# schulter/crbm

Hardware: AMD Instinct MI355X
Metric: Gibbs-steps/sec (PCD-1) at batch 8192x4x200, 10 motifs len 15 (higher is better)
Workload: dtype f32; 1 GPU; cfg2: 10 motifs len 15, batch 8192 x 4x200, PCD-1, single-stranded; chains_per_gpu=8192, gibbs_steps_per_launch=1, visible=4x200, hidden=10x186, parallelism=chains sharded over 1 GPU(s), no collective in the Gibbs step

## Files before the change

__graft_entry__.py:

```python
import os
import sys

ROOT = os.path.dirname(os.path.abspath(__file__))
if ROOT not in sys.path:
    sys.path.insert(0, ROOT)


PRECOMPILE = [dict(num_motifs=k, motif_length=m, doublestranded=ds) for (k, m, ds) in [
    (10, 15, 0), (10, 15, 1), (50, 25, 0), (20, 15, 1),
    (10, 5, 1), (10, 5, 0), (3, 4, 1), (4, 5, 1), (4, 5, 0), (6, 9, 1), (2, 5, 1),
]]
PRECOMPILE += [dict(num_motifs=6, motif_length=7, doublestranded=1, pooling=2, fantasy_hidden_len=24),
               dict(num_motifs=10, motif_length=15, doublestranded=0, pooling=4, fantasy_hidden_len=48),
               dict(num_motifs=5, motif_length=8, doublestranded=1, pooling=3, fantasy_hidden_len=36)]
PRECOMPILE += [dict(num_motifs=100, motif_length=15, doublestranded=0), dict(num_motifs=20, motif_length=40, doublestranded=1)]
PRECOMPILE += [dict(num_motifs=300, motif_length=10, doublestranded=0, fantasy_hidden_len=51), dict(num_motifs=120, motif_length=40, doublestranded=1, fantasy_hidden_len=61),
               dict(num_motifs=256, motif_length=4, doublestranded=1, fantasy_hidden_len=37), dict(num_motifs=300, motif_length=10, doublestranded=0, batchsize=4096, fantasy_hidden_len=191)]
PRECOMPILE += [dict(num_motifs=300, motif_length=10, doublestranded=0, batchsize=512, fantasy_hidden_len=30),
               dict(num_motifs=120, motif_length=40, doublestranded=1, batchsize=256, fantasy_hidden_len=24)]
PRECOMPILE += [dict(num_motifs=10, motif_length=15, doublestranded=0, batchsize=8192, fantasy_hidden_len=186),
               dict(num_motifs=50, motif_length=25, doublestranded=0, batchsize=8192, fantasy_hidden_len=976),
               dict(num_motifs=20, motif_length=15, doublestranded=1, batchsize=8192, fantasy_hidden_len=486)]
PRECOMPILE += [dict(num_motifs=3, motif_length=3, doublestranded=1, batchsize=4, fantasy_hidden_len=8),
               dict(num_motifs=4, motif_length=4, doublestranded=0, batchsize=4, fantasy_hidden_len=8)]

STATISTICS_SHAPES = [dict(num_motifs=k, motif_length=m, doublestranded=ds, pooling=pool, batchsize=7, fantasy_hidden_len=lf)
                     for (k, m, ds, pool, lf) in [
    (10, 15, 0, 1, 33), (16, 16, 1, 1, 33), (16, 32, 0, 1, 33), (32, 16, 0, 1, 33), (8, 12, 1, 1, 33), (20, 15, 1, 1, 33),
    (33, 17, 0, 1, 33), (64, 32, 1, 1, 33), (20, 40, 1, 1, 33), (4, 64, 1, 1, 33), (100, 15, 0, 1, 33), (130, 7, 1, 1, 33),
    (256, 4, 0, 1, 33), (6, 7, 1, 2, 34), (10, 15, 0, 4, 36), (5, 8, 1, 3, 33), (300, 10, 0, 1, 33), (150, 6, 1, 2, 34),
    (10, 15, 0, 1, 64), (10, 15, 0, 1, 32), (20, 40, 1, 1, 64), (20, 40, 1, 1, 32)]]
GEOMETRY_SHAPES = [dict(num_motifs=k, motif_length=m, doublestranded=ds, batchsize=b, fantasy_hidden_len=lf,
                        env=dict(CRBM_GEOM="2", CRBM_GIBBS_S=str(s)))
                   for (k, m, ds, lf, b, s) in [(10, 15, 0, 186, 8, 4), (10, 15, 0, 185, 8, 4), (10, 15, 0, 185, 6, 2), (10, 15, 1, 50, 6, 2), (40, 6, 0, 30, 4, 4),
                                                (10, 15, 0, 186, 9, 4), (10, 15, 1, 50, 8, 2)]]


def build():
    from crbm_amd.csrc import build as hip_build
    hip_build.build(verbose=True)
    hip_build.prune_cache()
    hip_build.precompile(PRECOMPILE + STATISTICS_SHAPES + GEOMETRY_SHAPES, verbose=False)
    from oracle import build_cpu
    build_cpu.build(verbose=True)
    import crbm_amd
    from crbm_amd import _lib
    lib = _lib.load()
    assert lib.crbm_abi_version() == _lib.ABI_VERSION
    print("crbm_amd", crbm_amd.__version__, "ABI", lib.crbm_abi_version())


def smoke():
    import numpy as np
    from crbm_amd import CRBM
    from oracle.crbm_oracle import OracleCRBM, synthetic_onehot

    K, M, B, Lf, n, L = 10, 15, 64, 186, 48, 200
    W = np.random.default_rng(42).standard_normal((K, 1, 4, M)).astype(np.float32)
    model = CRBM(K, M, doublestranded=False, batchsize=B, cd_k=1, fantasy_hidden_len=Lf, seed=2026)
    oracle = OracleCRBM(K, M, doublestranded=False, batchsize=B, cd_k=1, fantasy_hidden_len=Lf, seed=2026, W=W)
    b = (oracle.b + 4.0).astype(np.float32)
    model.motifs.set_value(W)
    model.bias.set_value(b)
    oracle.b = b.astype(np.float64)
    D = synthetic_onehot(n, L, seed=1234)
    model._trainingFct(D)
    oracle.train_step(D)
    np.testing.assert_allclose(model.motifs.get_value(), oracle.W, rtol=1e-4, atol=2e-6)
    np.testing.assert_allclose(model.bias.get_value(), oracle.b, rtol=1e-4, atol=2e-6)
    np.testing.assert_allclose(model.c.get_value(), oracle.c, rtol=1e-4, atol=2e-6)
    from oracle.crbm_oracle import hidden_uniforms, visible_uniforms, KIND_CHAIN_H, KIND_CHAIN_V
    model.set_fantasy(oracle.fantasy_h.astype(np.float32))
    idx = np.arange(B) + oracle.seq_offset
    for _ in range(3):
        t = oracle.gibbs_step
        model.set_rng(gibbs_step=t)
        uv = visible_uniforms(oracle.seed, t, idx, Lf + M - 1, KIND_CHAIN_V)
        Pv, v = oracle._computeVgivenH(oracle.fantasy_h, None, uv)
        uh = hidden_uniforms(oracle.seed, t, idx, K, Lf, 0, KIND_CHAIN_H)
        P, hnew = oracle._computeHgivenV(v, False, uh)
        model.gibbsSteps(1)
        h, _ = model.get_fantasy()
        gv = model.get_fantasy_visible()
        badv = (gv != v).any(axis=2)[:, 0]
        if badv.any():
            gap = np.min(np.abs(np.cumsum(Pv[:, 0], axis=1)[:, :3] - uv[:, None, :]), axis=1)
            assert np.all(gap[badv] < 1e-6), "visible sample differs away from a tie"
        bad = (h != hnew) & ~badv.any(axis=1)[:, None, None, None]
        assert np.all(np.abs(P - uh)[bad] < 1e-6), "hidden sample differs away from a tie"
        oracle.fantasy_h, oracle.gibbs_step = hnew, t + 1
        model.set_fantasy(hnew.astype(np.float32))
    assert oracle.fantasy_h.sum() > 0
    np.testing.assert_allclose(model.freeEnergy(D), oracle.freeEnergy(D), rtol=1e-4)
    print("smoke ok: train step, Gibbs chain and free energy match the oracle")


if __name__ == "__main__":
    build()
    if os.path.exists("/dev/kfd"):
        smoke()
```

crbm_amd/csrc/crbm_kernels.h:

```cpp
#pragma once
#include <hip/hip_runtime.h>
#include <stdint.h>
#include "crbm_layout.h"

namespace crbm {

template <int I>
struct IC {
  static constexpr int value = I;
};

struct Philox4 {
  uint32_t v[4];
};

struct HalfFrag {
  uint32_t r[4];
};
#if defined(__clang__)
typedef float floatx4 __attribute__((ext_vector_type(4)));
__device__ __forceinline__ uint32_t xor3(uint32_t a, uint32_t b, uint32_t c) { return __builtin_amdgcn_bitop3_b32(a, b, c, 0x96); }
__device__ __forceinline__ uint32_t bitrev32(uint32_t x) { return __builtin_bitreverse32(x); }
__device__ __forceinline__ void store4_streaming(uint32_t* dst, uint32_t x, uint32_t y, uint32_t z, uint32_t w) {
  typedef uint32_t u4v __attribute__((ext_vector_type(4)));
  const u4v val = {x, y, z, w};
  __builtin_nontemporal_store(val, reinterpret_cast<u4v*>(dst));
}
__device__ __forceinline__ void store1_streaming(uint32_t* dst, uint32_t x) { __builtin_nontemporal_store(x, dst); }
__device__ __forceinline__ void wait_vector_memory() { __builtin_amdgcn_s_waitcnt(0x0F70); }
__device__ __forceinline__ float load_system(const float* p) { return __hip_atomic_load(p, __ATOMIC_RELAXED, __HIP_MEMORY_SCOPE_SYSTEM); }
__device__ __forceinline__ uint32_t load_system(const uint32_t* p) { return __hip_atomic_load(p, __ATOMIC_RELAXED, __HIP_MEMORY_SCOPE_SYSTEM); }
__device__ __forceinline__ void store_system(float* p, float v) { __hip_atomic_store(p, v, __ATOMIC_RELAXED, __HIP_MEMORY_SCOPE_SYSTEM); }
__device__ __forceinline__ void store_system(uint32_t* p, uint32_t v) { __hip_atomic_store(p, v, __ATOMIC_RELAXED, __HIP_MEMORY_SCOPE_SYSTEM); }
__device__ __forceinline__ void fence_system() { __threadfence_system(); }
__device__ __forceinline__ void fence_acquire_system() { __builtin_amdgcn_fence(__ATOMIC_ACQUIRE, ""); }
__device__ __forceinline__ uint32_t ticket_add(uint32_t* p) { return __hip_atomic_fetch_add(p, 1u, __ATOMIC_ACQ_REL, __HIP_MEMORY_SCOPE_AGENT); }
__device__ __forceinline__ void short_sleep() { __builtin_amdgcn_s_sleep(8); }
__device__ __forceinline__ uint64_t realtime_ticks() { return __builtin_amdgcn_s_memrealtime(); }
__device__ __forceinline__ uint64_t shader_cycles() { return __builtin_amdgcn_s_memtime(); }
__device__ __forceinline__ void split_f16(const float (&x)[8], HalfFrag& hi, HalfFrag& lo) {
  typedef _Float16 half8 __attribute__((ext_vector_type(8)));
  half8 h, l;
#pragma unroll
  for (int e = 0; e < 8; ++e) {
    h[e] = (_Float16)x[e];
    l[e] = (_Float16)(x[e] - (float)h[e]);
  }
  hi = __builtin_bit_cast(HalfFrag, h);
  lo = __builtin_bit_cast(HalfFrag, l);
}
__device__ __forceinline__ floatx4 mfma_16x16x32_f16(const HalfFrag& a, const HalfFrag& b, floatx4 c) {
  typedef _Float16 half8 __attribute__((ext_vector_type(8)));
  return __builtin_amdgcn_mfma_f32_16x16x32_f16(__builtin_bit_cast(half8, a), __builtin_bit_cast(half8, b), c, 0, 0, 0);
}
typedef float floatx2 __attribute__((vector_size(8)));
__device__ __forceinline__ floatx2 fma2(floatx2 a, floatx2 b, floatx2 c) { return __builtin_elementwise_fma(a, b, c); }
__device__ __forceinline__ floatx2 opaque(floatx2 v) { asm volatile("" : "+v"(v)); return v; }
__device__ __forceinline__ uint32_t lanes_below(unsigned long long mask) {
  return __builtin_amdgcn_mbcnt_hi((uint32_t)(mask >> 32), __builtin_amdgcn_mbcnt_lo((uint32_t)mask, 0u));
}
#else
typedef float floatx4 __attribute__((vector_size(16)));
typedef float floatx2 __attribute__((vector_size(8)));
__device__ __forceinline__ floatx2 fma2(floatx2 a, floatx2 b, floatx2 c) { return floatx2{fmaf(a[0], b[0], c[0]), fmaf(a[1], b[1], c[1])}; }
__device__ __forceinline__ floatx2 opaque(floatx2 v) { return v; }
__device__ __forceinline__ uint32_t xor3(uint32_t a, uint32_t b, uint32_t c) { return a ^ b ^ c; }
__device__ __forceinline__ uint32_t bitrev32(uint32_t x) {
  x = ((x >> 1) & 0x55555555u) | ((x & 0x55555555u) << 1);
  x = ((x >> 2) & 0x33333333u) | ((x & 0x33333333u) << 2);
  x = ((x >> 4) & 0x0F0F0F0Fu) | ((x & 0x0F0F0F0Fu) << 4);
  x = ((x >> 8) & 0x00FF00FFu) | ((x & 0x00FF00FFu) << 8);
  return (x >> 16) | (x << 16);
}
__device__ __forceinline__ void store4_streaming(uint32_t* dst, uint32_t x, uint32_t y, uint32_t z, uint32_t w) {
  *reinterpret_cast<uint4*>(dst) = make_uint4(x, y, z, w);
}
__device__ __forceinline__ void store1_streaming(uint32_t* dst, uint32_t x) { *dst = x; }
__device__ __forceinline__ void wait_vector_memory() {}
__device__ __forceinline__ float load_system(const float* p) { float v; __atomic_load(p, &v, __ATOMIC_RELAXED); return v; }
__device__ __forceinline__ uint32_t load_system(const uint32_t* p) { return __atomic_load_n(p, __ATOMIC_RELAXED); }
__device__ __forceinline__ void store_system(float* p, float v) { __atomic_store(p, &v, __ATOMIC_RELAXED); }
__device__ __forceinline__ void store_system(uint32_t* p, uint32_t v) { __atomic_store_n(p, v, __ATOMIC_RELAXED); }
__device__ __forceinline__ void fence_system() { __atomic_thread_fence(__ATOMIC_SEQ_CST); }
__device__ __forceinline__ void fence_acquire_system() { __atomic_thread_fence(__ATOMIC_ACQUIRE); }
__device__ __forceinline__ uint32_t ticket_add(uint32_t* p) { return __atomic_fetch_add(p, 1u, __ATOMIC_ACQ_REL); }
__device__ __forceinline__ void short_sleep() {}
__device__ __forceinline__ uint64_t realtime_ticks() { return emu::realtime_ticks(); }
__device__ __forceinline__ uint64_t shader_cycles() { return emu::realtime_ticks(); }
__device__ __forceinline__ void split_f16(const float (&x)[8], HalfFrag& hi, HalfFrag& lo) { emu::split_f16(x, hi.r, lo.r); }
__device__ __forceinline__ uint32_t lanes_below(unsigned long long mask) {
  return (uint32_t)__popcll(mask & ((1ull << (threadIdx.x & 63u)) - 1ull));
}
}
unsigned long long atomicMax(unsigned long long* p, unsigned long long v);
namespace crbm {
__device__ __forceinline__ floatx4 mfma_16x16x32_f16(const HalfFrag& a, const HalfFrag& b, floatx4 c) {
  float d[4] = {c[0], c[1], c[2], c[3]};
  emu::mfma_16x16x32_f16(a.r, b.r, d);
  return floatx4{d[0], d[1], d[2], d[3]};
}
#endif

#ifndef CRBM_PHILOX_ROUNDS
#define CRBM_PHILOX_ROUNDS 7
#endif
__device__ __forceinline__ Philox4 philox4x32(uint32_t c0, uint32_t c1, uint32_t c2, uint32_t c3,
                                                 uint32_t k0, uint32_t k1) {
#pragma unroll
  for (int r = 0; r < CRBM_PHILOX_ROUNDS; ++r) {
    const uint64_t p0 = (uint64_t)0xD2511F53u * c0;
    const uint64_t p1 = (uint64_t)0xCD9E8D57u * c2;
    const uint32_t n0 = xor3((uint32_t)(p1 >> 32), c1, k0);
    const uint32_t n2 = xor3((uint32_t)(p0 >> 32), c3, k1);
    c1 = (uint32_t)p1;
    c3 = (uint32_t)p0;
    c0 = n0;
    c2 = n2;
    k0 += 0x9E3779B9u;
    k1 += 0xBB67AE85u;
  }
  Philox4 o;
  o.v[0] = c0; o.v[1] = c1; o.v[2] = c2; o.v[3] = c3;
  return o;
}

__device__ __forceinline__ uint32_t philox_pick(const Philox4& r, int i) {
  const uint32_t lo = (i & 1) ? r.v[1] : r.v[0];
  const uint32_t hi = (i & 1) ? r.v[3] : r.v[2];
  return (i & 2) ? hi : lo;
}

template <int I>
__device__ __forceinline__ uint32_t philox_field12(const Philox4& r) {
  constexpr int w = (12 * I) / 32, b = (12 * I) % 32;
  if (b <= 20) return (r.v[w] >> b) & 0xFFFu;
  return ((r.v[w] >> b) | (r.v[(w + 1) & 3] << ((32 - b) & 31))) & 0xFFFu;
}

__device__ __forceinline__ uint32_t philox_field12_dyn(const Philox4& r, int i) {
  const int b = 12 * i, w = b >> 5, sh = b & 31;
  uint32_t v = philox_pick(r, w) >> sh;
  if (sh > 20) v |= philox_pick(r, (w + 1) & 3) << (32 - sh);
  return v & 0xFFFu;
}

__device__ __forceinline__ float u01(uint32_t r) { return (float)(r >> 8) * 5.9604644775390625e-8f; }

__device__ __forceinline__ uint32_t rng_word2(uint32_t kind, uint32_t strand, uint32_t sub, uint32_t group) {
  return (kind << 28) | (strand << 24) | (sub << 16) | group;
// ... 232 lines not shown
#pragma unroll 1
  for (int j = 0; j < POOL; ++j) {
    zfun(g0 + j, z);
#pragma unroll
    for (int k = 0; k < KP; ++k) zmin[k] = fminf(zmin[k], z[k]);
  }
  float den[KP];
#pragma unroll
  for (int k = 0; k < KP; ++k) { den[k] = (float)POOL * __builtin_amdgcn_exp2f(zmin[k]); cb[k] = 0.f; p[k] = 0.f; }
#pragma unroll 1
  for (int j = 0; j < POOL; ++j) {
    zfun(g0 + j, z);
#pragma unroll
    for (int k = 0; k < KP; ++k) {
      const float e = __builtin_amdgcn_exp2f(zmin[k] - z[k]);
      den[k] += e;
      cb[k] += j < me ? e : 0.f;
      p[k] = j == me ? e : p[k];
    }
  }
#pragma unroll
  for (int k = 0; k < KP; ++k) {
    const float inv = 1.0f / den[k];
    S[k] = (den[k] - (float)POOL * __builtin_amdgcn_exp2f(zmin[k])) * inv;
    p[k] *= inv;
    cb[k] *= inv;
  }
}

template <class C>
__device__ __forceinline__ void hidden_uniforms24(uint32_t n, uint32_t s, uint32_t kind, uint32_t strand, const RngView& rng,
                                                  uint32_t step, float (&u)[C::KP], uint32_t group0 = 0) {
#pragma unroll
  for (int g = 0; g < C::NGRP; ++g) {
    const Philox4 rc = philox4x32(n, s, rng_word2(kind, strand, 0, group0 + (uint32_t)g), step, rng.seed_lo, rng.seed_hi);
    const Philox4 rf = philox4x32(n, s, rng_word2(kind, strand, 1, group0 + (uint32_t)g), step, rng.seed_lo, rng.seed_hi);
    auto unit = [&](auto I) {
      constexpr int i = decltype(I)::value;
      const int k = 10 * g + i;
      if (k < C::K) u[k] = (float)(philox_field12<i>(rc) * 4096u + philox_field12<i>(rf)) * 5.9604644775390625e-8f;
    };
    unit(IC<0>{}); unit(IC<1>{}); unit(IC<2>{}); unit(IC<3>{}); unit(IC<4>{});
    unit(IC<5>{}); unit(IC<6>{}); unit(IC<7>{}); unit(IC<8>{}); unit(IC<9>{});
  }
}

template <int POOL, int KP, class ZFun>
__device__ __forceinline__ void pooled_softplus(ZFun zfun, int g0, float (&acc)[KP], int nvalid) {
  float zmin[KP], z[KP], den[KP];
#pragma unroll
  for (int k = 0; k < KP; ++k) zmin[k] = 0.f;
#pragma unroll 1
  for (int j = 0; j < POOL; ++j) {
    zfun(g0 + j, z);
#pragma unroll
    for (int k = 0; k < KP; ++k) zmin[k] = fminf(zmin[k], z[k]);
  }
#pragma unroll
  for (int k = 0; k < KP; ++k) den[k] = __builtin_amdgcn_exp2f(zmin[k]);
#pragma unroll 1
  for (int j = 0; j < POOL; ++j) {
    zfun(g0 + j, z);
#pragma unroll
    for (int k = 0; k < KP; ++k) den[k] += __builtin_amdgcn_exp2f(zmin[k] - z[k]);
  }
#pragma unroll
  for (int k = 0; k < KP; ++k)
    if (k < nvalid) acc[k] += 0.6931471805599453f * (__builtin_amdgcn_logf(den[k]) - zmin[k]);
}

template <class C>
__device__ __forceinline__ void pooled_sample(const float (&p)[C::KP], const float (&cb)[C::KP], const float (&u)[C::KP],
                                              uint32_t (&mask)[C::NW]) {
#pragma unroll
  for (int w = 0; w < C::NW; ++w) mask[w] = 0u;
#pragma unroll
  for (int k = 0; k < C::K; ++k) {
    const uint32_t one = (cb[k] + p[k] > u[k] && cb[k] <= u[k]) ? 1u : 0u;
    mask[k >> 5] |= one << (k & 31);
  }
}

template <int NFLOATS>
__device__ __forceinline__ void copy_tables(float* dst, const float* src) {
  static_assert(NFLOATS % 4 == 0, "tables are float4 granular");
  const float4* s4 = reinterpret_cast<const float4*>(src);
  float4* d4 = reinterpret_cast<float4*>(dst);
  for (int i = threadIdx.x; i < NFLOATS / 4; i += blockDim.x) d4[i] = s4[i];
}

constexpr float LOG2E = 1.4426950408889634f, LN2 = 0.6931471805599453f;
struct TablesArgs {
  const float* W;
  const float* b;
  const float* c;
  float* out;
};

template <class C, int LIMIT = C::TABLES_ALL>
__device__ void build_tables_range(const TablesArgs& a, int first, int stride) {
  constexpr int K = C::K, M = C::M;
  for (int idx = first; idx < LIMIT; idx += stride) {
    float val = 0.f;
    if (idx < C::TAB) {
      const int t0 = idx;
      const int k = t0 % C::KP, r = (t0 / C::KP) % C::ROWS, g = t0 / (C::KP * C::ROWS);
      if (k < K) {
        for (int t = 0; t < C::G; ++t) {
          const int j = g * C::G + t;
          if (j < M) {
            const int al = (r >> (2 * t)) & 3;
            val += a.W[(k * 4 + al) * M + j];
          }
        }
        if (g == 0) val += a.b[k];
        val *= -LOG2E;
      } else if (g == 0) {
        val = 1e30f;
      }
    } else if (idx < C::OFF_C) {
      const bool rc = C::DS && idx >= C::OFF_TVR;
      const int t0 = idx - (rc ? C::OFF_TVR : C::OFF_TV);
      const int al = t0 & 3, pat = (t0 >> 2) & 31, ch = (t0 >> 7) % C::NCH, jr = (t0 >> 7) / C::NCH;
      for (int bit = 0; bit < 5; ++bit) {
        const int k = 5 * ch + bit;
        if (k < K && ((pat >> bit) & 1))
          val += rc ? a.W[(k * 4 + (3 - al)) * M + jr] : a.W[(k * 4 + al) * M + (M - 1 - jr)];
      }
      val *= LOG2E;
    } else if (idx < C::TABLES) {
      val = LOG2E * a.c[idx - C::OFF_C];
    } else if (idx < C::OFF_C2) {
      const bool rc = C::DS && idx >= C::OFF_WSR;
      const int t0 = idx - (rc ? C::OFF_WSR : C::OFF_WS);
      const int al = t0 & 3, k = (t0 >> 2) % K, jr = (t0 >> 2) / K - 4;
      if (jr >= 0 && jr < M) val = LOG2E * (rc ? a.W[(k * 4 + (3 - al)) * M + jr] : a.W[(k * 4 + al) * M + (M - 1 - jr)]);
    } else {
      val = LOG2E * a.c[idx - C::OFF_C2];
    }
    a.out[idx] = val;
  }
}

template <class C>
__device__ void build_tables_body(const TablesArgs& a) {
  build_tables_range<C>(a, (int)(blockIdx.x * blockDim.x + threadIdx.x), (int)(gridDim.x * blockDim.x));
}
template <class C>
__device__ void build_gather_table_body(const TablesArgs& a) {
  build_tables_range<C, C::TAB>(a, (int)(blockIdx.x * blockDim.x + threadIdx.x), (int)(gridDim.x * blockDim.x));
}

struct HgvArgs {
  const float* tables;
  const uint32_t* letters;
  int32_t n, L, Lh, LW;
  int32_t TS;
  FastDiv divLh;
  int32_t mode;
  float* act;
  float* prob;
  float* sample;
  unsigned long long* ones;
  RngView rng;
  uint32_t kind;
};

struct HgvMasksArgs {
  HgvArgs g;
  uint32_t* masks;
  int32_t NWfull, k0, Kfull, kskip;
// ... 443 lines not shown
      if constexpr (C::POOL > 1) {
        if (valid) {
          const uint32_t* lrow = a.letters + (size_t)chain * a.LW;
          constexpr int NV = 4 * R::NQW;
          float p[NV], cb[NV], S[NV];
#pragma unroll
          for (int strand = 0; strand <= C::DS; ++strand) {
            auto zfun = [&](int pos, float (&z)[NV]) {
              const LetterWin<M> w = letter_window<M>(lrow, pos);
              conv_gather_quads<C, R::NQW>(Tf, strand ? revcomp_window<M>(w) : w, 4 * nt0, z);
            };
            pooled_probs<C::POOL, NV>(zfun, s, p, cb, S);
#pragma unroll
            for (int kl = 0; kl < KW; ++kl)
              if (16 * nt0 + kl < K) {
                const float ps = 16384.0f * p[kl];
                col[(size_t)(strand * KW + kl) * STATS_RS] = ps;
                if (SP && strand == 0) col[(size_t)((1 + C::DS) * KW + kl) * STATS_RS] = ps * (1.0f - S[kl]);
              }
          }
        } else {
#pragma unroll
          for (int r = 0; r < R::PARKED * KW; ++r) col[(size_t)r * STATS_RS] = 0.f;
        }
      } else
      if (valid) {
        const LetterWin<M> wl = letter_window<M>(gw + NPW * slot, e);
        float z[4 * R::NQW];
        conv_gather_quads<C, R::NQW>(Tf, wl, 4 * nt0, z);
#pragma unroll
        for (int kl = 0; kl < KW; ++kl)
          if (16 * nt0 + kl < K) {
            const float ps = fast_rcp(fmaf(exp_neg_x(z[kl]), STATS_PSCALE_INV, STATS_PSCALE_INV));
            col[(size_t)kl * STATS_RS] = ps;
            if (SP && !R::QDERIVE) col[(size_t)((1 + C::DS) * KW + kl) * STATS_RS] = fmaf(-ps * STATS_PSCALE_INV, ps, ps);
          }
        if (C::DS) {
          conv_gather_quads<C, R::NQW>(Tf, revcomp_window<M>(wl), 4 * nt0, z);
#pragma unroll
          for (int kl = 0; kl < KW; ++kl)
            if (16 * nt0 + kl < K)
              col[(size_t)(KW + kl) * STATS_RS] = fast_rcp(fmaf(exp_neg_x(z[kl]), STATS_PSCALE_INV, STATS_PSCALE_INV));
        }
      } else {
#pragma unroll
        for (int r = 0; r < R::PARKED * KW; ++r) col[(size_t)r * STATS_RS] = 0.f;
      }
    }
    __builtin_amdgcn_wave_barrier();
#pragma unroll
    for (int slot = 0; slot < 2; ++slot)
      if (G0 + slot < ngroups && !(a.debug & 1))
        stats_mfma_group<C, R, BYTE_LUT>(Pt, win + 2 * NPW * slot, lut, nt0, slot, acc);
    __builtin_amdgcn_wave_barrier();
  }
  if (a.debug & 8) return;
  stats_mfma_finish<C, SP>(sg, smem, nt0, bid, acc, vcount);
}

struct GibbsArgs {
  const float* tables;
  const float* tables_tf = nullptr;
  int32_t off_ws = 0;
  uint32_t* hm;
  uint32_t* hmp;
  uint32_t* vout;
  int32_t nchains, Lf, Lv, S;
  int32_t nvb, nhb;
  int32_t Lrow;
  int32_t LWs;
  FastDiv divVB, divHB, divRow, divLfw;
  int32_t steps;
  RngView rng;
  uint32_t* ones;
  unsigned long long* clock = nullptr;
  unsigned long long* timeline = nullptr;
  int32_t debug;
  int32_t nblocks;
  int32_t stats_off;
  StatsGeom sg;
};

struct GeomRT {
  static constexpr bool CT = false, PROF = true, ALIGNED = false, ONE = false;
  const GibbsArgs& a;
  __device__ __forceinline__ explicit GeomRT(const GibbsArgs& a_) : a(a_) {}
  __device__ __forceinline__ int S() const { return a.S; }
  __device__ __forceinline__ int Lf() const { return a.Lf; }
  __device__ __forceinline__ int Lv() const { return a.Lv; }
  __device__ __forceinline__ int Lrow() const { return a.Lrow; }
  __device__ __forceinline__ int LWs() const { return a.LWs; }
  __device__ __forceinline__ int nvb() const { return a.nvb; }
  __device__ __forceinline__ int nhb() const { return a.nhb; }
  __device__ __forceinline__ int nchains() const { return a.nchains; }
  __device__ __forceinline__ uint32_t threads() const { return blockDim.x; }
  __device__ __forceinline__ int nblk() const { return a.nblocks > 0 ? a.nblocks : (int)gridDim.x; }
  __device__ __forceinline__ uint32_t div_vb(uint32_t i) const { return fastdiv_tile(i, a.divVB); }
  __device__ __forceinline__ uint32_t div_hb(uint32_t i) const { return fastdiv_tile(i, a.divHB); }
  template <int NW> __device__ __forceinline__ uint32_t div_lfw(uint32_t i) const { return fastdiv_tile(i, a.divLfw); }
};
template <int S_, int LF_, int LV_, int LROW_, int LWS_, int NVB_, int NHB_, int TB_, int NCHAINS_, int GRID_, bool ALIGNED_>
struct GeomCT {
  static_assert(S_ >= 1 && NCHAINS_ % S_ == 0 && GRID_ >= 1 && GRID_ <= NCHAINS_ / S_ && TB_ % 64 == 0, "GeomCT: full tiles only");
  static constexpr bool CT = true, PROF = false, ALIGNED = ALIGNED_, ONE = GRID_ == NCHAINS_ / S_;
  __device__ __forceinline__ explicit GeomCT(const GibbsArgs&) {}
  __device__ __forceinline__ constexpr int S() const { return S_; }
  __device__ __forceinline__ constexpr int Lf() const { return LF_; }
  __device__ __forceinline__ constexpr int Lv() const { return LV_; }
  __device__ __forceinline__ constexpr int Lrow() const { return LROW_; }
  __device__ __forceinline__ constexpr int LWs() const { return LWS_; }
  __device__ __forceinline__ constexpr int nvb() const { return NVB_; }
  __device__ __forceinline__ constexpr int nhb() const { return NHB_; }
  __device__ __forceinline__ constexpr int nchains() const { return NCHAINS_; }
  __device__ __forceinline__ constexpr uint32_t threads() const { return TB_; }
  __device__ __forceinline__ constexpr int nblk() const { return GRID_; }
  __device__ __forceinline__ uint32_t div_vb(uint32_t i) const { return i / (uint32_t)NVB_; }
  __device__ __forceinline__ uint32_t div_hb(uint32_t i) const { return i / (uint32_t)NHB_; }
  template <int NW> __device__ __forceinline__ uint32_t div_lfw(uint32_t i) const { return i / (uint32_t)(LF_ * NW); }
};

__device__ __forceinline__ uint32_t sample_letter(float y0, float y1, float y2, float y3, float u) {
  const float mx = fmaxf(fmaxf(y0, y1), fmaxf(y2, y3));
  const float e0 = __builtin_amdgcn_exp2f(y0 - mx), e1 = __builtin_amdgcn_exp2f(y1 - mx), e2 = __builtin_amdgcn_exp2f(y2 - mx),
              e3 = __builtin_amdgcn_exp2f(y3 - mx);
  const float t = u * ((e0 + e1) + (e2 + e3));
  return (uint32_t)(t >= e0) + (uint32_t)(t >= e0 + e1) + (uint32_t)(t >= (e0 + e1) + e2);
}

template <class C>
__device__ __forceinline__ void topdown_bits(unsigned long long w, const char* tab, int q_base, float (&y)[4][4], int unit_base = 0) {
  constexpr int K = C::K;
  const char* tab_q = tab + ((size_t)q_base * K + unit_base) * 16;
  const char* idle = tab - K * 16;
  auto rows_of = [&](unsigned long long bits) { return bits ? tab_q + (__ffsll(bits) - 1) * 16 : idle; };
  auto fetch = [&](const char* p, float4 (&t)[4]) {
#pragma unroll
    for (int i = 0; i < 4; ++i) t[i] = *reinterpret_cast<const float4*>(p + (4 - i) * K * 16);
  };
  float4 cur[4];
  fetch(rows_of(w), cur);
  while (w) {
    w &= w - 1ull;
    float4 nxt[4];
    fetch(rows_of(w), nxt);
#pragma unroll
    for (int i = 0; i < 4; ++i) {
      y[i][0] += cur[i].x; y[i][1] += cur[i].y; y[i][2] += cur[i].z; y[i][3] += cur[i].w;
      cur[i] = nxt[i];
    }
  }
}

template <class C, bool SPARSE, bool STATS = false, class GP = GeomRT>
__device__ void gibbs_body(const GibbsArgs& a, int bid = -1) {
  const GP g(a);
  const int dbg = GP::PROF ? a.debug : 0;
  const uint32_t TB = g.threads();
  constexpr int KP = C::KP, M = C::M, NW = C::NW, NCH = C::NCH;
  static_assert(SPARSE || C::DENSE, "no dense top-down tables for this model");
  using SR = StatsRole<C, false>;
  static_assert(!STATS || SR::NR == 1, "the fused statistics need all motifs of a position in one wave");
  constexpr int LTAB = SPARSE ? C::SP_TABLES : C::TABLES;
  HIP_DYNAMIC_SHARED(float, smem);
  const float* Tf = smem;
  const float* cv = smem + (SPARSE ? C::SP_C : C::OFF_C);
  uint32_t* hm = reinterpret_cast<uint32_t*>(smem + LTAB);
  uint32_t* hmp = hm + (size_t)g.S() * g.Lrow() * NW;
  uint32_t* let = hmp + (C::DS ? (size_t)g.S() * g.Lrow() * NW : 0);
  uint32_t* fixq = let + (size_t)g.S() * g.LWs();
#ifdef CRBM_INLINE_EXACT_PATH
  constexpr bool DEFER = false;
#else
  constexpr bool DEFER = C::POOL == 1 && C::DS;
#endif

  bool tables_done = (dbg & 1) != 0;
  auto copy_all_tables = [&]() {
    if (SPARSE) {
      copy_tables<C::TAB>(smem, a.tables_tf ? a.tables_tf : a.tables);
      copy_tables<C::WS * (1 + C::DS) + 4>(smem + C::SP_WS, a.tables + (a.tables_tf ? a.off_ws : C::OFF_WS));
    } else {
      copy_tables<C::TABLES>(smem, a.tables);
    }
    tables_done = true;
  };

  const int rowW = g.Lrow() * NW;
  const uint32_t per = (uint32_t)(g.Lf() * NW);
  const int ntiles = (g.nchains() + g.S() - 1) / g.S();
  if (bid < 0) bid = (int)blockIdx.x;
  if constexpr (GP::PROF) {
    if (a.clock && bid == 0 && threadIdx.x == 0) {
      a.clock[2] = realtime_ticks();
      a.clock[3] = shader_cycles();
    }
    if (a.timeline && bid == 0 && threadIdx.x == 0) a.timeline[0] = realtime_ticks();
  }
  const int nblk = g.nblk();
  int nset = 0;
  const int lane = threadIdx.x & 63, wave = threadIdx.x >> 6, nwaves = TB >> 6;
  float* sreg = nullptr;
  uint32_t* swin = nullptr;
  float* sPt = nullptr;
  floatx4 sacc[STATS ? SR::NACC : 1];
  float vcount = 0.f;
  if constexpr (STATS) {
    sreg = smem + a.stats_off;
    float* sslice = sreg + a.sg.off_slices + (size_t)wave * a.sg.slice;
    swin = reinterpret_cast<uint32_t*>(sslice + a.sg.off_win);
    sPt = sslice + a.sg.off_pt;
#pragma unroll
    for (int t = 0; t < SR::NACC; ++t) sacc[t] = floatx4{0.f, 0.f, 0.f, 0.f};
    stats_build_lut<false>(reinterpret_cast<uint32_t*>(sreg));
    for (int i = lane; i < SR::ROWS * STATS_RS; i += 64) sPt[i] = 0.f;
  }
  if (threadIdx.x == 0) fixq[0] = 0u;
  {
    const int padw = rowW - (int)per, front = (M - 1) * NW;
    for (int idx = threadIdx.x; idx < g.S() * padw; idx += TB) {
      const int nl = idx / padw, e = idx - nl * padw;
      const int d = nl * rowW + (e < front ? e : e + (int)per);
      hm[d] = 0u;
      if (C::DS) hmp[d] = 0u;
    }
  }
  for (int tile = bid; GP::ONE ? tile == bid : tile < ntiles; tile += nblk) {
    const int n0 = tile * g.S();
    const int ns = GP::CT ? g.S() : min(g.S(), g.nchains() - n0);
    __syncthreads();
    if (!(dbg & 2)) {
      const uint32_t nwords = (uint32_t)ns * per;
      auto lds_index = [&](uint32_t i) {
        const uint32_t nl = g.template div_lfw<NW>(i);
        return nl * (uint32_t)rowW + (uint32_t)((M - 1) * NW) + (i - nl * per);
      };
      const size_t g0 = (size_t)n0 * per;
      if (GP::CT ? GP::ALIGNED : ((g0 | nwords) & 3u) == 0u) {
        constexpr int UN = 2;
        const uint4* src = reinterpret_cast<const uint4*>(a.hm + g0);
        const uint4* srcp = C::DS ? reinterpret_cast<const uint4*>(a.hmp + g0) : nullptr;
        for (uint32_t base0 = 0; base0 < nwords / 4; base0 += UN * TB) {
          const uint32_t base = base0 + threadIdx.x;
          uint4 t[UN], tp[UN];
#pragma unroll
          for (int u = 0; u < UN; ++u) {
            const uint32_t i4 = base + u * TB;
            if (i4 < nwords / 4) {
              t[u] = src[i4];
              if (C::DS) tp[u] = srcp[i4];
            }
          }
          if (!tables_done) copy_all_tables();
#pragma unroll
          for (int u = 0; u < UN; ++u) {
            const uint32_t i4 = base + u * TB;
            if (i4 < nwords / 4) {
              const uint32_t e[4] = {t[u].x, t[u].y, t[u].z, t[u].w};
              const uint32_t ep[4] = {tp[u].x, tp[u].y, tp[u].z, tp[u].w};
#pragma unroll
              for (int c = 0; c < 4; ++c) {
                const uint32_t d = lds_index(4 * i4 + c);
                hm[d] = e[c];
                if (C::DS) hmp[d] = ep[c];
              }
            }
// ... 14 lines not shown
          }
          if (!tables_done) copy_all_tables();
#pragma unroll
          for (int u = 0; u < UN; ++u) {
            const uint32_t i = base + u * TB;
            if (i < nwords) {
              const uint32_t d = lds_index(i);
              hm[d] = t[u];
              if (C::DS) hmp[d] = tp[u];
            }
          }
        }
      }
    }
    if (!tables_done) copy_all_tables();
    for (int idx = threadIdx.x; idx < ns * g.LWs(); idx += TB) let[idx] = 0u;
    auto resolve = [&](uint32_t e, int st, bool last) -> uint32_t {
      const uint32_t it = e & 0xFFFFFu, k = (e >> 20) & 0x7FFu, strand = e >> 31;
      const uint32_t nl = g.div_hb(it);
      const int s = (int)(it - nl * (uint32_t)g.nhb());
      const uint32_t gn = a.rng.seq_offset + (uint32_t)(n0 + nl);
      LetterWin<M> win = letter_window<M>(let + nl * (uint32_t)g.LWs(), s);
      if (strand) win = revcomp_window<M>(win);
      const float* T = Tf + k;
      float z = 0.f;
#pragma unroll
      for (int g = 0; g < C::NG; ++g) {
        const uint32_t r = window_bits<C::M>(win, 2 * C::G * g) & (uint32_t)(C::ROWS - 1);
        const float t = T[((size_t)g * C::ROWS + r) * KP];
        z = g == 0 ? t : z + t;
      }
      const uint32_t g10 = k / 10u, i10 = k - 10u * g10, step = a.rng.step + (uint32_t)st;
      const Philox4 rc = philox4x32(gn, (uint32_t)s, rng_word2(KIND_CHAIN_H, strand, 0, g10), step, a.rng.seed_lo, a.rng.seed_hi);
      const Philox4 rf = philox4x32(gn, (uint32_t)s, rng_word2(KIND_CHAIN_H, strand, 1, g10), step, a.rng.seed_lo, a.rng.seed_hi);
      const float t = 4096.0f * fast_rcp(1.0f + exp_neg_x(z));
      const float frac = t - (float)philox_field12_dyn(rc, (int)i10);
      const uint32_t one = frac * 4096.0f > (float)philox_field12_dyn(rf, (int)i10) ? 1u : 0u;
      if (one) {
        const uint32_t bit = 1u << (k & 31u), w = k >> 5;
        if (last) { if (!(dbg & 4)) atomicOr((strand ? a.hmp : a.hm) + (size_t)n0 * per + it * (uint32_t)NW + w, bit); }
        else atomicOr((strand ? hmp : hm) + (nl * (uint32_t)(rowW - (int)per) + it * (uint32_t)NW + (uint32_t)((M - 1) * NW)) + w, bit);
      }
      return one;
    };
    auto defer_units = [&](const uint32_t (&pending)[C::NGRP], uint32_t it, uint32_t strand, int st, bool last) -> uint32_t {
      uint32_t any = 0u, ones = 0u;
#pragma unroll
      for (int g = 0; g < C::NGRP; ++g) any |= pending[g];
      if (__any(any != 0u)) {
#pragma unroll
        for (int g = 0; g < C::NGRP; ++g) {
          uint32_t m = pending[g];
          while (m) {
            const uint32_t i = (uint32_t)__ffs(m) - 1u;
            m &= m - 1u;
            const uint32_t e = it | ((10u * (uint32_t)g + i) << 20) | (strand << 31);
            const uint32_t slot = atomicAdd(&fixq[0], 1u);
            if (slot < (uint32_t)FIXQ_CAP) fixq[2 + slot] = e;
            else ones += resolve(e, st, last);
          }
        }
      }
      return ones;
    };
    auto drain_queue = [&](int st, bool last) {
      if (last) wait_vector_memory();
      __syncthreads();
      const uint32_t nq = min(fixq[0], (uint32_t)FIXQ_CAP);
      for (uint32_t e = threadIdx.x; e < nq; e += TB) {
        const uint32_t one = resolve(fixq[2 + e], st, last);
        if (last) nset += (int)one;
      }
    };
    for (int st = 0; st < a.steps; ++st) {
      __syncthreads();
      if (threadIdx.x == 0) fixq[0] = 0u;
      for (uint32_t it = threadIdx.x; it < (uint32_t)(ns * g.nvb()); it += TB) {
        const uint32_t nl = g.div_vb(it);
        const int pb = (int)(it - nl * (uint32_t)g.nvb());
        const int p0 = 4 * pb;
        float y[4][4];
#pragma unroll
        for (int i = 0; i < 4; ++i) { y[i][0] = cv[0]; y[i][1] = cv[1]; y[i][2] = cv[2]; y[i][3] = cv[3]; }
        if constexpr (!SPARSE) {
          constexpr int NMV = (M + 3 + 3) / 4;
#pragma unroll
          for (int strand = 0; strand <= C::DS; ++strand) {
            const uint4* mrow = reinterpret_cast<const uint4*>((strand ? hmp : hm) + (size_t)nl * g.Lrow() + p0);
            const char* Tv = reinterpret_cast<const char*>(smem + (strand ? C::OFF_TVR : C::OFF_TV));
            uint32_t off[4 * NMV][NCH];
#pragma unroll
            for (int v4 = 0; v4 < NMV; ++v4) {
              const uint4 mm = mrow[v4];
              const uint32_t m4[4] = {mm.x, mm.y, mm.z, mm.w};
#pragma unroll
              for (int e = 0; e < 4; ++e)
#pragma unroll
                for (int ch = 0; ch < NCH; ++ch)
                  off[4 * v4 + e][ch] = (5 * ch >= 4 ? (m4[e] >> (5 * ch - 4)) : (m4[e] << (4 - 5 * ch))) & 0x1F0u;
            }
#pragma unroll
            for (int jr = 0; jr < M; ++jr)
#pragma unroll
              for (int ch = 0; ch < NCH; ++ch)
#pragma unroll
                for (int i = 0; i < 4; ++i) {
                  const float4 t = *reinterpret_cast<const float4*>(Tv + (jr * NCH + ch) * 512 + off[i + jr][ch]);
                  y[i][0] += t.x; y[i][1] += t.y; y[i][2] += t.z; y[i][3] += t.w;
                }
          }
        } else {
          constexpr int NSLOT = M + 3;
          constexpr int PPW = NW == 1 ? 64 / C::K : 1;
          constexpr int NWORD = (NSLOT + PPW - 1) / PPW;
#pragma unroll
          for (int strand = 0; strand <= C::DS; ++strand) {
            const uint32_t* mrow = (strand ? hmp : hm) + ((size_t)nl * g.Lrow() + p0) * NW;
            const char* tab = reinterpret_cast<const char*>(smem + (strand ? C::SP_WSR : C::SP_WS));
            if constexpr (NW == 1) {
              constexpr int NMV = (NSLOT + 3) / 4;
              uint32_t m[4 * NMV];
#pragma unroll
              for (int v4 = 0; v4 < NMV; ++v4) {
                const uint4 mm = reinterpret_cast<const uint4*>(mrow)[v4];
                m[4 * v4] = mm.x; m[4 * v4 + 1] = mm.y; m[4 * v4 + 2] = mm.z; m[4 * v4 + 3] = mm.w;
              }
#pragma unroll
              for (int wi = 0; wi < NWORD; ++wi) {
                unsigned long long w = 0ull;
#pragma unroll
                for (int t = 0; t < PPW; ++t)
                  if (wi * PPW + t < NSLOT) w |= (unsigned long long)m[wi * PPW + t] << (t * C::K);
                topdown_bits<C>(w, tab, wi * PPW, y);
              }
            } else {
#pragma unroll 1
              for (int q = 0; q < NSLOT; ++q) {
                if constexpr (NW == 2) {
                  const uint2 mm = *reinterpret_cast<const uint2*>(mrow + 2 * q);
                  topdown_bits<C>((unsigned long long)mm.x | ((unsigned long long)mm.y << 32), tab, q, y);
                } else {
#pragma unroll
                  for (int w2 = 0; 2 * w2 < NW; ++w2) {
                    const uint32_t lo = mrow[NW * q + 2 * w2], hi = 2 * w2 + 1 < NW ? mrow[NW * q + 2 * w2 + 1] : 0u;
                    topdown_bits<C>((unsigned long long)lo | ((unsigned long long)hi << 32), tab, q, y, 64 * w2);
                  }
                }
              }
            }
          }
        }
        const Philox4 r = philox4x32(a.rng.seq_offset + (uint32_t)(n0 + nl), (uint32_t)pb,
                                        rng_word2(KIND_CHAIN_V, 0, 0, 0), a.rng.step + (uint32_t)st,
                                        a.rng.seed_lo, a.rng.seed_hi);
        uint32_t byte = 0u;
#pragma unroll
        for (int i = 0; i < 4; ++i) {
          const uint32_t l = sample_letter(y[i][0], y[i][1], y[i][2], y[i][3], u01(r.v[i]));
          byte |= (p0 + i < g.Lv() ? l : 0u) << (2 * i);
        }
        reinterpret_cast<unsigned char*>(let + (size_t)nl * g.LWs())[pb] = (unsigned char)byte;
      }
      __syncthreads();
      bool fused_pass = false;
      if constexpr (STATS) if (st == a.steps - 1) {
        fused_pass = true;
        constexpr int KW = SR::KW;
        const int GPC = a.sg.GPC, ngl = ns * GPC;
        for (int u = wave; 2 * u < ngl; u += nwaves) {
          const int G0 = 2 * u;
          constexpr int NPW = C::NPW;
          if (lane < 8 * NPW) {
            const int G = G0 + lane / (4 * NPW), w = (lane >> 2) % NPW;
            int gi = 0;
            uint32_t word = 0u;
            if (G < ngl) {
              const uint32_t nl = fastdiv_tile((uint32_t)G, a.sg.divGPC);
              gi = G - (int)nl * GPC;
              if (2 * gi + w < g.LWs()) word = let[(size_t)nl * g.LWs() + 2 * gi + w];
            }
            vcount += stats_window_piece<NPW>(reinterpret_cast<unsigned short*>(swin), lane, word, G < ngl, gi, GPC, g.Lv());
          }
          __builtin_amdgcn_wave_barrier();
          {
            const int slot = lane >> 5, G = G0 + slot;
            bool valid = G < ngl;
            uint32_t nl = 0u;
            int s = 0;
            if (valid) {
              nl = fastdiv_tile((uint32_t)G, a.sg.divGPC);
              s = 32 * (G - (int)nl * GPC) + (lane & 31);
              valid = s < g.Lf();
            }
            float* col = sPt + lane;
            if (valid) {
              const uint32_t gn = a.rng.seq_offset + (uint32_t)(n0 + nl);
              const LetterWin<M> win = letter_window<M>(let + (size_t)nl * g.LWs(), s);
#pragma unroll
              for (int strand = 0; strand <= C::DS; ++strand) {
                float x[KP], p[KP];
                conv_gather<C>(Tf, strand ? revcomp_window<M>(win) : win, x);
                uint32_t mask[NW];
                uint32_t pend[C::NGRP];
                sample_hidden<C, 2, DEFER>(x, gn, (uint32_t)s, KIND_CHAIN_H, (uint32_t)strand, a.rng,
                                           a.rng.step + (uint32_t)st, mask, p, pend);
                uint32_t* dst = (strand ? a.hmp : a.hm) + (size_t)(n0 + nl) * per + (size_t)s * NW;
#pragma unroll
                for (int w = 0; w < NW; ++w) {
                  if (!(dbg & 4)) store1_streaming(dst + w, mask[w]);
                  nset += __popc(mask[w]);
                }
                if constexpr (DEFER) nset += (int)defer_units(pend, nl * (uint32_t)g.nhb() + (uint32_t)s, (uint32_t)strand, st, true);
#pragma unroll
                for (int k = 0; k < C::K; ++k) col[(size_t)(strand * KW + k) * STATS_RS] = p[k];
              }
            } else {
#pragma unroll
              for (int r = 0; r < SR::KINDS * KW; ++r) col[(size_t)r * STATS_RS] = 0.f;
            }
          }
          __builtin_amdgcn_wave_barrier();
#pragma unroll
          for (int slot = 0; slot < 2; ++slot)
            if (G0 + slot < ngl)
              stats_mfma_group<C, SR, false>(sPt, swin + 2 * C::NPW * slot, reinterpret_cast<const uint32_t*>(sreg), 0, slot, sacc);
          __builtin_amdgcn_wave_barrier();
        }
      }
      if (!fused_pass) {
      for (uint32_t it = threadIdx.x; it < (uint32_t)(ns * g.nhb()); it += TB) {
        const uint32_t nl = g.div_hb(it);
        const int s = (int)(it - nl * (uint32_t)g.nhb());
        const uint32_t gn = a.rng.seq_offset + (uint32_t)(n0 + nl);
        const uint32_t* lrow = let + nl * (uint32_t)g.LWs();
        const LetterWin<M> win = letter_window<M>(lrow, s);
#pragma unroll
        for (int strand = 0; strand <= C::DS; ++strand) {
          float x[KP], p[KP];
          uint32_t mask[NW], pend[C::NGRP];
          if constexpr (C::POOL > 1) {
            auto zfun = [&](int pos, float (&z)[KP]) {
              const LetterWin<M> w = letter_window<M>(lrow, pos);
              conv_gather<C>(Tf, strand ? revcomp_window<M>(w) : w, z);
// ... 1813 lines not shown
```

Measured before the change: 64580 8192-chain batch Gibbs steps/s (summed over GPUs).

## Tighten visible sampling: branchless letter packing, asm mask packing, batched table copy

```diff
diff --git a/__graft_entry__.py b/__graft_entry__.py
--- a/__graft_entry__.py
+++ b/__graft_entry__.py
@@ -35,12 +35,15 @@
                    for (k, m, ds, lf, b, s) in [(10, 15, 0, 186, 8, 4), (10, 15, 0, 185, 8, 4), (10, 15, 0, 185, 6, 2), (10, 15, 1, 50, 6, 2), (40, 6, 0, 30, 4, 4),
                                                 (10, 15, 0, 186, 9, 4), (10, 15, 1, 50, 8, 2)]]
 
+GOLDEN_SHAPES = [dict(num_motifs=k, motif_length=5, doublestranded=0, batchsize=4, fantasy_hidden_len=20,
+                      env=dict(CRBM_GEOM="2", CRBM_GIBBS_S="2")) for k in (7, 16, 21)]
+
 
 def build():
     from crbm_amd.csrc import build as hip_build
     hip_build.build(verbose=True)
     hip_build.prune_cache()
-    hip_build.precompile(PRECOMPILE + STATISTICS_SHAPES + GEOMETRY_SHAPES, verbose=False)
+    hip_build.precompile(PRECOMPILE + STATISTICS_SHAPES + GEOMETRY_SHAPES + GOLDEN_SHAPES, verbose=False)
     from oracle import build_cpu
     build_cpu.build(verbose=True)
     import crbm_amd
diff --git a/crbm_amd/csrc/crbm_kernels.h b/crbm_amd/csrc/crbm_kernels.h
--- a/crbm_amd/csrc/crbm_kernels.h
+++ b/crbm_amd/csrc/crbm_kernels.h
@@ -21,6 +21,26 @@
 typedef float floatx4 __attribute__((ext_vector_type(4)));
 __device__ __forceinline__ uint32_t xor3(uint32_t a, uint32_t b, uint32_t c) { return __builtin_amdgcn_bitop3_b32(a, b, c, 0x96); }
 __device__ __forceinline__ uint32_t bitrev32(uint32_t x) { return __builtin_bitreverse32(x); }
+template <int SH>
+__device__ __forceinline__ uint32_t shl_or(uint32_t x, uint32_t acc) {
+#if defined(__HIP_DEVICE_COMPILE__)
+  uint32_t r;
+  asm("v_lshl_or_b32 %0, %1, %2, %3" : "=v"(r) : "v"(x), "n"(SH), "v"(acc));
+  return r;
+#else
+  return (x << SH) | acc;
+#endif
+}
+__device__ __forceinline__ float max4_finite(float a, float b, float c, float d) {
+#if defined(__HIP_DEVICE_COMPILE__)
+  float m, r;
+  asm("v_max3_f32 %0, %1, %2, %3" : "=v"(m) : "v"(a), "v"(b), "v"(c));
+  asm("v_max_f32 %0, %1, %2" : "=v"(r) : "v"(m), "v"(d));
+  return r;
+#else
+  return fmaxf(fmaxf(a, b), fmaxf(c, d));
+#endif
+}
 __device__ __forceinline__ void store4_streaming(uint32_t* dst, uint32_t x, uint32_t y, uint32_t z, uint32_t w) {
   typedef uint32_t u4v __attribute__((ext_vector_type(4)));
   const u4v val = {x, y, z, w};
@@ -65,6 +85,8 @@
 __device__ __forceinline__ floatx2 fma2(floatx2 a, floatx2 b, floatx2 c) { return floatx2{fmaf(a[0], b[0], c[0]), fmaf(a[1], b[1], c[1])}; }
 __device__ __forceinline__ floatx2 opaque(floatx2 v) { return v; }
 __device__ __forceinline__ uint32_t xor3(uint32_t a, uint32_t b, uint32_t c) { return a ^ b ^ c; }
+__device__ __forceinline__ float max4_finite(float a, float b, float c, float d) { return fmaxf(fmaxf(a, b), fmaxf(c, d)); }
+template <int SH> __device__ __forceinline__ uint32_t shl_or(uint32_t x, uint32_t acc) { return (x << SH) | acc; }
 __device__ __forceinline__ uint32_t bitrev32(uint32_t x) {
   x = ((x >> 1) & 0x55555555u) | ((x & 0x55555555u) << 1);
   x = ((x >> 2) & 0x33333333u) | ((x & 0x33333333u) << 2);
@@ -463,11 +485,34 @@
 }
 
 template <int NFLOATS>
-__device__ __forceinline__ void copy_tables(float* dst, const float* src) {
+__device__ __forceinline__ void copy_tables(float* dst, const float* src, uint32_t stride) {
   static_assert(NFLOATS % 4 == 0, "tables are float4 granular");
   const float4* s4 = reinterpret_cast<const float4*>(src);
   float4* d4 = reinterpret_cast<float4*>(dst);
-  for (int i = threadIdx.x; i < NFLOATS / 4; i += blockDim.x) d4[i] = s4[i];
+  for (uint32_t i = threadIdx.x; i < (uint32_t)(NFLOATS / 4); i += stride) d4[i] = s4[i];
+}
+template <int NFLOATS>
+__device__ __forceinline__ void copy_tables(float* dst, const float* src) { copy_tables<NFLOATS>(dst, src, blockDim.x); }
+template <int NA, int NB, int TB>
+__device__ __forceinline__ void copy_tables_batched(float* dstA, const float* srcA, float* dstB, const float* srcB) {
+  static_assert(NA % 4 == 0 && NB % 4 == 0, "tables are float4 granular");
+  constexpr int A4 = NA / 4, B4 = NB / 4, RA = (A4 + TB - 1) / TB, RB = (B4 + TB - 1) / TB, R = RA + RB, CAP = 8;
+  const float4 *sA = reinterpret_cast<const float4*>(srcA), *sB = reinterpret_cast<const float4*>(srcB);
+  float4 *dA = reinterpret_cast<float4*>(dstA), *dB = reinterpret_cast<float4*>(dstB);
+#pragma unroll
+  for (int j0 = 0; j0 < R; j0 += CAP) {
+    float4 v[CAP];
+    int at[CAP];
+#pragma unroll
+    for (int c = 0; c < CAP; ++c) {
+      const int j = j0 + c, r = j < RA ? j : j - RA, n4 = j < RA ? A4 : B4, i = r * TB + (int)threadIdx.x;
+      at[c] = (r + 1) * TB <= n4 ? i : min(i, n4 - 1);
+      if (j < R) v[c] = (j < RA ? sA : sB)[at[c]];
+    }
+#pragma unroll
+    for (int c = 0; c < CAP; ++c)
+      if (j0 + c < R) (j0 + c < RA ? dA : dB)[at[c]] = v[c];
+  }
 }
 
 constexpr float LOG2E = 1.4426950408889634f, LN2 = 0.6931471805599453f;
@@ -1077,7 +1122,8 @@
 };
 
 struct GeomRT {
-  static constexpr bool CT = false, PROF = true, ALIGNED = false, ONE = false;
+  static constexpr bool CT = false, PROF = true, ALIGNED = false, ONE = false, WHOLE_BYTES = false;
+  static constexpr int TB = 0;
   const GibbsArgs& a;
   __device__ __forceinline__ explicit GeomRT(const GibbsArgs& a_) : a(a_) {}
   __device__ __forceinline__ int S() const { return a.S; }
@@ -1098,6 +1144,8 @@
 struct GeomCT {
   static_assert(S_ >= 1 && NCHAINS_ % S_ == 0 && GRID_ >= 1 && GRID_ <= NCHAINS_ / S_ && TB_ % 64 == 0, "GeomCT: full tiles only");
   static constexpr bool CT = true, PROF = false, ALIGNED = ALIGNED_, ONE = GRID_ == NCHAINS_ / S_;
+  static constexpr bool WHOLE_BYTES = LV_ % 4 == 0;
+  static constexpr int TB = TB_;
   __device__ __forceinline__ explicit GeomCT(const GibbsArgs&) {}
   __device__ __forceinline__ constexpr int S() const { return S_; }
   __device__ __forceinline__ constexpr int Lf() const { return LF_; }
@@ -1114,12 +1162,37 @@
   template <int NW> __device__ __forceinline__ uint32_t div_lfw(uint32_t i) const { return i / (uint32_t)(LF_ * NW); }
 };
 
-__device__ __forceinline__ uint32_t sample_letter(float y0, float y1, float y2, float y3, float u) {
-  const float mx = fmaxf(fmaxf(y0, y1), fmaxf(y2, y3));
+__device__ __forceinline__ uint32_t push_letter(uint32_t acc, float y0, float y1, float y2, float y3, float u) {
+  const float mx = max4_finite(y0, y1, y2, y3);
   const float e0 = __builtin_amdgcn_exp2f(y0 - mx), e1 = __builtin_amdgcn_exp2f(y1 - mx), e2 = __builtin_amdgcn_exp2f(y2 - mx),
               e3 = __builtin_amdgcn_exp2f(y3 - mx);
   const float t = u * ((e0 + e1) + (e2 + e3));
-  return (uint32_t)(t >= e0) + (uint32_t)(t >= e0 + e1) + (uint32_t)(t >= (e0 + e1) + e2);
+  const float da = t - e0, db = t - (e0 + e1), dc = t - ((e0 + e1) + e2);
+  acc = shift_in_sign(acc, db);
+  return (acc << 1) | (xor3(__float_as_uint(da), __float_as_uint(db), __float_as_uint(dc)) >> 31);
+}
+__device__ __forceinline__ uint32_t sample_letter(float y0, float y1, float y2, float y3, float u) {
+  return ~push_letter(0u, y0, y1, y2, y3, u) & 3u;
+}
+template <bool FULL>
+__device__ __forceinline__ uint32_t letter_byte(uint32_t inv, int p0, int Lv) {
+  if constexpr (FULL) return ~inv & 0xFFu;
+  else return ~inv & (0xFFu >> (2 * max(0, 4 - (Lv - p0))));
+}
+
+template <int K, int T, int N>
+__device__ __forceinline__ void pack_masks(const uint32_t* m, int n, uint32_t& lo, uint32_t& hi) {
+  if constexpr (T < N) {
+    constexpr int o = T * K;
+    if (T < n) {
+      if constexpr (o == 0) lo = m[T];
+      else if constexpr (o < 32) lo = shl_or<o % 32>(m[T], lo);
+      if constexpr (o < 32 && o + K > 32) hi = m[T] >> ((32 - o) % 32);
+      else if constexpr (o == 32) hi = m[T];
+      else if constexpr (o > 32) hi = shl_or<(o - 32) % 32>(m[T], hi);
+    }
+    pack_masks<K, T + 1, N>(m, n, lo, hi);
+  }
 }
 
 template <class C>
@@ -1172,10 +1245,16 @@
   bool tables_done = (dbg & 1) != 0;
   auto copy_all_tables = [&]() {
     if (SPARSE) {
-      copy_tables<C::TAB>(smem, a.tables_tf ? a.tables_tf : a.tables);
-      copy_tables<C::WS * (1 + C::DS) + 4>(smem + C::SP_WS, a.tables + (a.tables_tf ? a.off_ws : C::OFF_WS));
+      const float* tf = a.tables_tf ? a.tables_tf : a.tables;
+      const float* ws = a.tables + (a.tables_tf ? a.off_ws : C::OFF_WS);
+      if constexpr (GP::CT && GP::ONE) {
+        copy_tables_batched<C::TAB, C::WS * (1 + C::DS) + 4, GP::CT ? GP::TB : 64>(smem, tf, smem + C::SP_WS, ws);
+      } else {
+        copy_tables<C::TAB>(smem, tf, TB);
+        copy_tables<C::WS * (1 + C::DS) + 4>(smem + C::SP_WS, ws, TB);
+      }
     } else {
-      copy_tables<C::TABLES>(smem, a.tables);
+      copy_tables<C::TABLES>(smem, a.tables, TB);
     }
     tables_done = true;
   };
@@ -1356,6 +1435,15 @@
         float y[4][4];
 #pragma unroll
         for (int i = 0; i < 4; ++i) { y[i][0] = cv[0]; y[i][1] = cv[1]; y[i][2] = cv[2]; y[i][3] = cv[3]; }
+        if constexpr (SPARSE) {
+#pragma unroll
+          for (int i = 1; i < 4; ++i)
+#pragma unroll
+            for (int h = 0; h < 2; ++h) {
+              const floatx2 pr = opaque(floatx2{y[i][2 * h], y[i][2 * h + 1]});
+              y[i][2 * h] = pr[0]; y[i][2 * h + 1] = pr[1];
+            }
+        }
         if constexpr (!SPARSE) {
           constexpr int NMV = (M + 3 + 3) / 4;
 #pragma unroll
@@ -1401,10 +1489,9 @@
               }
 #pragma unroll
               for (int wi = 0; wi < NWORD; ++wi) {
-                unsigned long long w = 0ull;
-#pragma unroll
-                for (int t = 0; t < PPW; ++t)
-                  if (wi * PPW + t < NSLOT) w |= (unsigned long long)m[wi * PPW + t] << (t * C::K);
+                uint32_t lo = 0u, hi = 0u;
+                pack_masks<C::K, 0, PPW>(m + wi * PPW, NSLOT - wi * PPW, lo, hi);
+                const unsigned long long w = (unsigned long long)lo | ((unsigned long long)hi << 32);
                 topdown_bits<C>(w, tab, wi * PPW, y);
               }
             } else {
@@ -1427,12 +1514,10 @@
         const Philox4 r = philox4x32(a.rng.seq_offset + (uint32_t)(n0 + nl), (uint32_t)pb,
                                         rng_word2(KIND_CHAIN_V, 0, 0, 0), a.rng.step + (uint32_t)st,
                                         a.rng.seed_lo, a.rng.seed_hi);
-        uint32_t byte = 0u;
-#pragma unroll
-        for (int i = 0; i < 4; ++i) {
-          const uint32_t l = sample_letter(y[i][0], y[i][1], y[i][2], y[i][3], u01(r.v[i]));
-          byte |= (p0 + i < g.Lv() ? l : 0u) << (2 * i);
-        }
+        uint32_t inv = 0u;
+#pragma unroll
+        for (int i = 3; i >= 0; --i) inv = push_letter(inv, y[i][0], y[i][1], y[i][2], y[i][3], u01(r.v[i]));
+        const uint32_t byte = letter_byte<GP::WHOLE_BYTES>(inv, p0, g.Lv());
         reinterpret_cast<unsigned char*>(let + (size_t)nl * g.LWs())[pb] = (unsigned char)byte;
       }
       __syncthreads();
```

New measurement: 67790 8192-chain batch Gibbs steps/s (summed over GPUs) (median of 6 runs). 1.05x the previous value.
